# althonos/pyrodigal

Hardware: AMD Instinct MI355X
Metric: Mbp/sec gene-called (meta mode) (higher is better)
Workload: dtype f64; 1 GPU; 100000x20kbp_gc30-70_meta; contigs=100000, bases=2000000000, models=16, contigs_rank0=100000, sub_batch_contigs=6250, contexts_per_gpu=4, genes_all_ranks=2908995, steps_issued=a join of the contexts and a gather per step

## Files before the change

pyrodigal_amd/csrc/finder.hip:

```cpp
#include "pga_internal.h"
#include "pipeline.h"
#include "dpw_core.h"
#include "dev_common.h"
#include "find_plan.h"

#include <math.h>
#include <stdio.h>
#include <stdlib.h>
#include <string.h>

#include <algorithm>
#include <atomic>
#include <chrono>
#include <condition_variable>
#include <functional>
#include <limits>
#include <map>
#include <memory>
#include <mutex>
#include <new>
#include <thread>
#include <type_traits>
#include <unordered_map>

// ... 451 lines not shown
    int64_t out_off;
    int64_t dp_off;
    int64_t fin_off;
    int64_t topo_off;
    int32_t n;
    int32_t _pad;
};
struct GcPtrs { const float* p[4]; };
struct OutArrays {
    int32_t* ndx; int32_t* stop_val; uint8_t* type; int8_t* strand; float* gc_cont;
    uint8_t* edge_dp; double* cscore_dp; double* sscore_dp; double* rscore_dp; double* uscore_dp; double* tscore_dp;
    int32_t* star_ptr; int32_t* traceb; int8_t* ov_mark; double* score;
    uint8_t* edge; double* cscore; double* sscore; double* rscore; double* uscore; double* tscore; double* mot_score;
    int32_t* mot_ndx; uint8_t* rbs; uint8_t* mot_len; uint8_t* mot_spacer; uint8_t* mot_spacendx;
    int32_t direct;
    const int32_t* g_ndx[4]; const int32_t* g_stop_val[4]; const uint8_t* g_type[4]; const int8_t* g_strand[4];
    const uint8_t* c_edge; const double* c_cscore; const double* c_rscore; const double* c_uscore; const double* c_tscore;
    const int32_t* c_star_ptr; const double* d_score;
};

__global__ void __launch_bounds__(256)
k_gather_winners(const WinDesc* __restrict__ wd, int n_win, int64_t out_begin, int64_t total, GroupArrays ga, ChainArrays ca,
                 DpBuffers dp, OutArrays o, const int lean ) {
    __shared__ int s_w0;
    const int64_t blk0 = out_begin + (int64_t)blockIdx.x * blockDim.x;
    const int64_t g = blk0 + threadIdx.x;
    int lo = block_search_le([&](const int k) { return wd[k].out_off; }, n_win, blk0, &s_w0);
    if (g >= out_begin + total) return;
    while (lo + 1 < n_win && wd[lo + 1].out_off <= g) lo++;
    const WinDesc w = wd[lo];
    const int i = (int)(g - w.out_off);
    const int64_t t = w.topo_off + i, a = w.dp_off + i, f = w.fin_off + i;
    if (o.direct) { o.sscore_dp[g] = ca.sscore[a]; o.traceb[g] = dp.traceb[a]; o.ov_mark[g] = dp.ov_mark[a]; return; }
    o.ndx[g] = ga.ndx[t]; o.stop_val[g] = ga.stop_val[t]; o.type[g] = ga.type[t]; o.strand[g] = ga.strand[t];
    o.edge_dp[g] = ca.edge[a]; o.cscore_dp[g] = ca.cscore[a]; o.sscore_dp[g] = ca.sscore[a]; o.rscore_dp[g] = ca.rscore[a];
    o.uscore_dp[g] = ca.uscore[a]; o.tscore_dp[g] = ca.tscore[a];
    o.star_ptr[3 * g] = ca.star_ptr[3 * a]; o.star_ptr[3 * g + 1] = ca.star_ptr[3 * a + 1]; o.star_ptr[3 * g + 2] = ca.star_ptr[3 * a + 2];
    o.traceb[g] = dp.traceb[a]; o.ov_mark[g] = dp.ov_mark[a]; o.score[g] = dp.score[a];
    if (lean) return;
    o.gc_cont[g] = ga.gc_cont[t];
    o.edge[g] = ca.edge[f]; o.cscore[g] = ca.cscore[f]; o.sscore[g] = ca.sscore[f]; o.rscore[g] = ca.rscore[f];
    o.uscore[g] = ca.uscore[f]; o.tscore[g] = ca.tscore[f]; o.mot_score[g] = ca.mot_score[f]; o.mot_ndx[g] = ca.mot_ndx[f];
    o.rbs[2 * g] = ca.rbs[2 * f]; o.rbs[2 * g + 1] = ca.rbs[2 * f + 1];
    o.mot_len[g] = ca.mot_len[f]; o.mot_spacer[g] = ca.mot_spacer[f]; o.mot_spacendx[g] = ca.mot_spacendx[f];
}

struct GeneNodeAttr {
    double cscore, sscore, rscore, uscore, tscore, mot_score;
    float gc_cont; int32_t mot_ndx;
    uint8_t edge, rbs0, rbs1, mot_len, mot_spacer, _pad[3];
};
__global__ void __launch_bounds__(256)
k_gather_gene_nodes(const int64_t* __restrict__ idx, int n, OutArrays o, GeneNodeAttr* __restrict__ out) {
    const int t = blockIdx.x * blockDim.x + threadIdx.x;
    if (t >= n) return;
    const int64_t g = idx[t];
    GeneNodeAttr a;
    a.cscore = o.cscore[g]; a.sscore = o.sscore[g]; a.rscore = o.rscore[g]; a.uscore = o.uscore[g]; a.tscore = o.tscore[g];
    a.mot_score = o.mot_score[g]; a.gc_cont = o.gc_cont[g]; a.mot_ndx = o.mot_ndx[g];
    a.edge = o.edge[g]; a.rbs0 = o.rbs[2 * g]; a.rbs1 = o.rbs[2 * g + 1]; a.mot_len = o.mot_len[g]; a.mot_spacer = o.mot_spacer[g];
    a._pad[0] = a._pad[1] = a._pad[2] = 0;
    out[t] = a;
}

__device__ inline NodeView node_view(const TailDesc& d, const OutArrays& o, int32_t* tracef, uint8_t* elim) {
    const int64_t oo = d.out_off;
    if (o.direct) {
        const int64_t t = d.topo_off, a = d.dp_off; const int g = d.group;
        return NodeView{d.n, o.g_ndx[g] + t, o.g_stop_val[g] + t, o.g_type[g] + t, o.g_strand[g] + t, o.c_edge + a,
                        const_cast<double*>(o.c_cscore) + a, o.sscore_dp + oo, o.c_rscore + a, o.c_uscore + a, o.c_tscore + a,
                        o.c_star_ptr + 3 * a, o.traceb + oo, tracef + oo, o.ov_mark + oo, o.d_score + a, elim + oo};
    }
    return NodeView{d.n, o.ndx + oo, o.stop_val + oo, o.type + oo, o.strand + oo, o.edge_dp + oo,
                    o.cscore_dp + oo, o.sscore_dp + oo, o.rscore_dp + oo, o.uscore_dp + oo, o.tscore_dp + oo,
                    o.star_ptr + 3 * oo, o.traceb + oo, tracef + oo, o.ov_mark + oo, o.score + oo, elim + oo};
}

__global__ void __launch_bounds__(64)
k_tail_path(const TailDesc* __restrict__ td, int n_contigs, OutArrays o, int32_t* tracef, uint8_t* elim, int32_t* __restrict__ path,
            GeneRec* __restrict__ genes, int32_t* __restrict__ n_genes) {
    const int i = blockIdx.x * blockDim.x + threadIdx.x;
    if (i >= n_contigs) return;
    const TailDesc d = td[i];
    int ng = 0;
    if (d.n > 0 && d.mx >= 0) {
        NodeView v = node_view(d, o, tracef, elim);
        int32_t* pl = path + d.out_off;
        const int cnt = untangle(v, d.mx, pl);
        if (v.traceb[d.mx] != -1) {
            eliminate_bad_genes(v, pl, cnt, d.st_wt);
            ng = extract_genes(v, pl, cnt, genes + d.gene_off);
        }
    }
    n_genes[i] = ng;
}

__device__ inline int contig_of_slot(const TailDesc* __restrict__ td, int n_contigs, int64_t slot) {
    int lo = 0, hi = n_contigs - 1;
    while (lo < hi) { const int mid = (lo + hi + 1) >> 1; if (td[mid].gene_off <= slot) lo = mid; else hi = mid - 1; }
    return lo;
}

__global__ void __launch_bounds__(256)
k_tail_tweak(const TailDesc* __restrict__ td, int n_contigs, int64_t n_slots, OutArrays o, int32_t* tracef, uint8_t* elim,
             const GeneRec* __restrict__ orig, GeneRec* __restrict__ out, const int32_t* __restrict__ n_genes, int maxov,
             uint8_t* __restrict__ changed, int32_t* __restrict__ n_changed) {
    const int64_t slot = (int64_t)blockIdx.x * blockDim.x + threadIdx.x;
    if (slot >= n_slots) return;
    const int c = contig_of_slot(td, n_contigs, slot);
    const TailDesc d = td[c];
    const int g = (int)(slot - d.gene_off), ng = n_genes[c];
    if (g >= ng) return;
    const NodeView v = node_view(d, o, tracef, elim);
    const GeneRec* base = orig + d.gene_off;
    GeneRec cur = base[g];
    tweak_one(v, g > 0 ? &base[g - 1] : nullptr, cur, g < ng - 1 ? &base[g + 1] : nullptr, d.st_wt, maxov);
    out[slot] = cur;
    const bool moved = cur.start_ndx != base[g].start_ndx && v.strand[cur.start_ndx] == -1;
    changed[slot] = moved ? 1 : 0;
    if (moved) atomicAdd(&n_changed[c], 1);
}
__global__ void __launch_bounds__(256)
k_tail_init(int32_t* __restrict__ tracef, uint8_t* __restrict__ elim, const int64_t n_nodes, int32_t* __restrict__ nchanged, int32_t* __restrict__ ngenes ,
            const int n_contigs, int32_t* __restrict__ seg_cnt , const int n_segs) {
    const int64_t t = (int64_t)blockIdx.x * blockDim.x + threadIdx.x, stride = (int64_t)gridDim.x * blockDim.x;
    for (int64_t k = t; k <= n_nodes; k += stride) { tracef[k] = -1; elim[k] = 0; }
    for (int64_t k = t; k <= n_contigs; k += stride) { nchanged[k] = 0; if (ngenes != nullptr) ngenes[k] = 0; }
    if (seg_cnt != nullptr) for (int64_t k = t; k < n_segs; k += stride) seg_cnt[k] = 0;
}

__global__ void __launch_bounds__(1024)
k_gene_prefix(const int32_t* __restrict__ n_genes, int n_contigs, int32_t* __restrict__ gpre) {
    __shared__ int s_w[16];
    __shared__ int s_carry;
    const int t = threadIdx.x, lane = t & 63, w = t >> 6;
    if (t == 0) s_carry = 0;
    __syncthreads();
    for (int base = 0; base < n_contigs; base += 1024) {
        const int v = base + t < n_contigs ? n_genes[base + t] : 0;
        int inc = v;
#pragma unroll
        for (int o = 1; o < 64; o <<= 1) { const int x = __shfl_up(inc, o, 64); if (lane >= o) inc += x; }
        if (lane == 63) s_w[w] = inc;
        __syncthreads();
        int run = s_carry + inc - v;
        for (int k = 0; k < w; k++) run += s_w[k];
        if (base + t < n_contigs) gpre[base + t] = run;
        __syncthreads();
        if (t == 1023) s_carry = run + v;
        __syncthreads();
    }
    if (t == 0) gpre[n_contigs] = s_carry;
}
__global__ void __launch_bounds__(256)
k_tail_tweak_packed(const TailDesc* __restrict__ td, int n_contigs, OutArrays o, int32_t* tracef, uint8_t* elim,
                    const GeneRec* __restrict__ orig, GeneRec* __restrict__ out, const int32_t* __restrict__ n_genes, int maxov,
                    uint8_t* __restrict__ changed, int32_t* __restrict__ n_changed, const int32_t* __restrict__ gpre) {
    const int total = gpre[n_contigs];
    for (int q = blockIdx.x * blockDim.x + threadIdx.x; q < total; q += gridDim.x * blockDim.x) {
        int lo = 0, hi = n_contigs - 1;
        while (lo < hi) { const int mid = (lo + hi + 1) >> 1; if (gpre[mid] <= q) lo = mid; else hi = mid - 1; }
        const int c = lo, g = q - gpre[c], ng = n_genes[c];
        const TailDesc d = td[c];
        const NodeView v = node_view(d, o, tracef, elim);
        const GeneRec* base = orig + d.gene_off;
        GeneRec cur = base[g];
        tweak_one(v, g > 0 ? &base[g - 1] : nullptr, cur, g < ng - 1 ? &base[g + 1] : nullptr, d.st_wt, maxov);
        out[d.gene_off + g] = cur;
        const bool moved = cur.start_ndx != base[g].start_ndx && v.strand[cur.start_ndx] == -1;
        changed[d.gene_off + g] = moved ? 1 : 0;
        if (moved) atomicAdd(&n_changed[c], 1);
    }
}
__device__ void tweak_one_wave(const NodeView& v, const GeneRec* prev, GeneRec& cur, const GeneRec* next, double w, int maxov, const int lane) {
    const int nn = v.n;
    const int ndx = cur.start_ndx;
    const double sc = v.sscore[ndx] + v.cscore[ndx];
    double ig = 0.0;
    const bool prev_fwd = prev && v.strand[prev->start_ndx] == 1, prev_rev = prev && v.strand[prev->start_ndx] == -1;
    const bool next_fwd = next && v.strand[next->start_ndx] == 1, next_rev = next && v.strand[next->start_ndx] == -1;
    if (v.strand[ndx] == 1 && prev_fwd) ig = igm_same_h(v, prev->stop_ndx, ndx, w);
    if (v.strand[ndx] == 1 && prev_rev) ig = -0.15 * w;
    if (v.strand[ndx] == -1 && next_fwd) ig = -0.15 * w;
    if (v.strand[ndx] == -1 && next_rev) ig = igm_same_h(v, ndx, next->stop_ndx, w);
    int mi[2] = {-1, -1}; double ms[2] = {0, 0}, mg[2] = {0, 0};
    const int sv_ndx = v.stop_val[ndx];
    for (int base = ndx - 100; base < ndx + 100; base += 64) {
        const int j = base + lane;
        bool cand = j >= 0 && j < nn && j != ndx && j < ndx + 100;
        double tg = 0.0, cs = 0.0;
        if (cand) cand = !(is_stop_n(v, j) | (v.stop_val[j] != sv_ndx));
        if (cand) {
            const int sj = v.strand[j];
            if (sj == 1 && prev_fwd) {
                if (v.ndx[prev->stop_ndx] - v.ndx[j] > maxov) cand = false;
                else tg = igm_same_h(v, prev->stop_ndx, j, w);
            }
            if (cand && sj == 1 && prev_rev) { if (v.ndx[prev->start_ndx] - v.ndx[j] >= 0) cand = false; else tg = -0.15 * w; }
            if (cand && sj == -1 && next_fwd) { if (v.ndx[j] - v.ndx[next->start_ndx] >= 0) cand = false; else tg = -0.15 * w; }
            if (cand && sj == -1 && next_rev) {
                if (v.ndx[j] - v.ndx[next->stop_ndx] > maxov) cand = false;
                else tg = igm_same_h(v, j, next->stop_ndx, w);
            }
            if (cand) cs = v.cscore[j] + v.sscore[j];
        }
        unsigned long long m = __ballot(cand);
        while (m) {
            const int k = __builtin_ctzll(m);
            m &= m - 1ull;
            const int jk = base + k;
            const double csk = __shfl(cs, k, 64), tgk = __shfl(tg, k, 64);
            if (mi[0] == -1) { mi[0] = jk; ms[0] = csk; mg[0] = tgk; }
            else if (csk + tgk > ms[0]) { mi[1] = mi[0]; ms[1] = ms[0]; mg[1] = mg[0]; mi[0] = jk; ms[0] = csk; mg[0] = tgk; }
            else if (mi[1] == -1 || csk + tgk > ms[1]) { mi[1] = jk; ms[1] = csk; mg[1] = tgk; }
        }
    }
    for (int k = 0; k < 2; k++) {
        const int m = mi[k];
        if (m == -1) continue;
        if (v.tscore[m] < v.tscore[ndx] && ms[k] - v.tscore[m] >= sc - v.tscore[ndx] + w && v.rscore[m] > v.rscore[ndx] &&
            v.uscore[m] > v.uscore[ndx] && v.cscore[m] > v.cscore[ndx] && abs(v.ndx[m] - v.ndx[ndx]) > 15) {
            ms[k] += v.tscore[ndx] - v.tscore[m];
        } else if (abs(v.ndx[m] - v.ndx[ndx]) <= 15 && v.rscore[m] + v.tscore[m] > v.rscore[ndx] + v.tscore[ndx] &&
                   v.edge[ndx] == 0 && v.edge[m] == 0) {
            if (v.cscore[ndx] > v.cscore[m]) ms[k] += v.cscore[ndx] - v.cscore[m];
            if (v.uscore[ndx] > v.uscore[m]) ms[k] += v.uscore[ndx] - v.uscore[m];
            if (ig > mg[k]) ms[k] += ig - mg[k];
        } else ms[k] = -1000.0;
    }
    int pick = -1;
    for (int k = 0; k < 2; k++) {
        if (mi[k] == -1) continue;
        if (pick == -1 && ms[k] + mg[k] > sc + ig) pick = k;
        else if (pick >= 0 && ms[k] + mg[k] > ms[pick] + mg[pick]) pick = k;
    }
    if (pick != -1 && v.strand[mi[pick]] == 1) { cur.start_ndx = mi[pick]; cur.begin = v.ndx[mi[pick]] + 1; }
    else if (pick != -1 && v.strand[mi[pick]] == -1) { cur.start_ndx = mi[pick]; cur.end = v.ndx[mi[pick]] + 1; }
}

__global__ void __launch_bounds__(256)
k_tail_tweak_wave(const TailDesc* __restrict__ td, int n_contigs, OutArrays o, int32_t* tracef, uint8_t* elim,
                  const GeneRec* __restrict__ orig, GeneRec* __restrict__ out, const int32_t* __restrict__ n_genes, int maxov,
                  uint8_t* __restrict__ changed, int32_t* __restrict__ n_changed) {
    const int c = blockIdx.y, lane = threadIdx.x & 63;
    const int g = blockIdx.x * 4 + (threadIdx.x >> 6), ng = n_genes[c];
    if (g >= ng) return;
    const TailDesc d = td[c];
    const NodeView v = node_view(d, o, tracef, elim);
    const GeneRec* base = orig + d.gene_off;
    GeneRec cur = base[g];
    GeneRec prev{}, nxt{};
    if (g > 0) prev = base[g - 1];
    if (g < ng - 1) nxt = base[g + 1];
    tweak_one_wave(v, g > 0 ? &prev : nullptr, cur, g < ng - 1 ? &nxt : nullptr, d.st_wt, maxov, lane);
    if (lane != 0) return;
    out[d.gene_off + g] = cur;
    const bool moved = cur.start_ndx != base[g].start_ndx && v.strand[cur.start_ndx] == -1;
    changed[d.gene_off + g] = moved ? 1 : 0;
    if (moved) atomicAdd(&n_changed[c], 1);
}

#define PGA_FIX_MAXWIN 4096
__global__ void __launch_bounds__(1024)
k_tail_tweak_fixup(const TailDesc* __restrict__ td, int n_contigs, OutArrays o, int32_t* tracef, uint8_t* elim,
                   const GeneRec* __restrict__ orig, const GeneRec* __restrict__ par_all, const int32_t* __restrict__ n_genes, int maxov,
                   const uint8_t* __restrict__ ch0_all, const int32_t* __restrict__ n_changed, GeneRec* __restrict__ fin_all,
                   uint8_t* __restrict__ chf_all) {
    __shared__ uint8_t s_redone[PGA_FIX_MAXWIN];
    const int c = blockIdx.x, lane = threadIdx.x & 63, wave = threadIdx.x >> 6, nwaves = blockDim.x >> 6;
    if (c >= n_contigs) return;
    const TailDesc d = td[c];
    const int ng = n_genes[c];
    const GeneRec* ob = orig + d.gene_off; const GeneRec* par = par_all + d.gene_off; const uint8_t* ch0 = ch0_all + d.gene_off;
    GeneRec* fin = fin_all + d.gene_off; uint8_t* chf = chf_all + d.gene_off;
    for (int g = threadIdx.x; g < ng; g += blockDim.x) { fin[g] = par[g]; chf[g] = ch0[g]; }
    if (n_changed[c] == 0 || ng < 2) return;
    __threadfence_block();
    __syncthreads();
    const NodeView v = node_view(d, o, tracef, elim);
    const int nwin = (ng - 1 + 63) >> 6;
    auto run_window = [&](const int w, const bool assume) -> bool {
        const int g0 = 1 + (w << 6), g1 = min(ng, g0 + 64);
        const int g = g0 + lane;
        if (!assume) {
            if (g < g1) { fin[g] = par[g]; chf[g] = ch0[g]; }
            __builtin_amdgcn_fence(__ATOMIC_RELEASE, "workgroup");
            __builtin_amdgcn_fence(__ATOMIC_ACQUIRE, "workgroup");
        }
        const int pf = g < g1 ? ((lane == 0 && !assume) ? chf[g - 1] : ch0[g - 1]) : 0;
        unsigned long long mask = __ballot(pf != 0);
        bool last = false;
        while (mask) {
            const int k = __builtin_ctzll(mask);
            mask &= mask - 1ull;
            const int gg = g0 + k;
            GeneRec cur = ob[gg];
            const GeneRec prev = (k == 0 && assume) ? par[gg - 1] : fin[gg - 1];
            GeneRec nxt{};
            if (gg < ng - 1) nxt = ob[gg + 1];
            tweak_one_wave(v, &prev, cur, gg < ng - 1 ? &nxt : nullptr, d.st_wt, maxov, lane);
            const int nf = cur.start_ndx != ob[gg].start_ndx && v.strand[cur.start_ndx] == -1;
            if (lane == 0) { fin[gg] = cur; chf[gg] = (uint8_t)nf; }
            __builtin_amdgcn_fence(__ATOMIC_RELEASE, "workgroup");
            __builtin_amdgcn_fence(__ATOMIC_ACQUIRE, "workgroup");
            if (gg + 1 < g1) { if (nf) mask |= 1ull << (k + 1); else mask &= ~(1ull << (k + 1)); }
            if (gg == g1 - 1) last = true;
        }
        return last;
    };
    if (nwin <= PGA_FIX_MAXWIN) {
        for (int w = wave; w < nwin; w += nwaves) { const bool r = run_window(w, true); if (lane == 0) s_redone[w] = r; }
        __threadfence_block();
        __syncthreads();
        if (wave == 0)
            for (int w = 1; w < nwin; w++)
                if (s_redone[w - 1]) { const bool r = run_window(w, false); if (lane == 0) s_redone[w] = r; __builtin_amdgcn_wave_barrier(); }
    } else if (wave == 0) {
        for (int w = 0; w < nwin; w++) run_window(w, false);
    }
}

__global__ void __launch_bounds__(256)
k_emit_genes(const TailDesc* __restrict__ td, int n_contigs, int64_t n_slots, OutArrays o, const GeneRec* __restrict__ fin,
             const int32_t* __restrict__ n_genes, const int64_t* __restrict__ gene_begin, int single, pga_gene* __restrict__ out,
             const int lean, ChainArrays ca, GcPtrs gcs) {
    const int64_t slot = (int64_t)blockIdx.x * blockDim.x + threadIdx.x;
    if (slot >= n_slots) return;
    const int c = contig_of_slot(td, n_contigs, slot);
    const TailDesc d = td[c];
    const int g = (int)(slot - d.gene_off);
    if (g >= n_genes[c]) return;
    const GeneRec gr = fin[slot];
    const int64_t sn = d.out_off + gr.start_ndx, en = d.out_off + gr.stop_ndx;
    pga_gene G;
    memset(&G, 0, sizeof G);
    G.contig = c; G.begin = gr.begin; G.end = gr.end; G.start_ndx = gr.start_ndx; G.stop_ndx = gr.stop_ndx;
    if (o.direct) {
        const int64_t ts = d.topo_off + gr.start_ndx, as = d.dp_off + gr.start_ndx, ae = d.dp_off + gr.stop_ndx;
        const int64_t fs = d.fin_off + gr.start_ndx, fe = d.fin_off + gr.stop_ndx;
        G.strand = o.g_strand[d.group][ts];
        const uint8_t se = single ? o.c_edge[as] : ca.edge[fs], ee = single ? o.c_edge[ae] : ca.edge[fe];
        G.partial_begin = G.strand == 1 ? se : ee; G.partial_end = G.strand == 1 ? ee : se;
        G.start_type = se ? 3 : o.g_type[d.group][ts];
        G.rbs[0] = ca.rbs[2 * fs]; G.rbs[1] = ca.rbs[2 * fs + 1];
        G.mot_len = ca.mot_len[fs]; G.mot_spacer = ca.mot_spacer[fs]; G.mot_ndx = ca.mot_ndx[fs]; G.mot_score = ca.mot_score[fs];
        G.gc_cont = gcs.p[d.group][ts];
        G.cscore = single ? o.c_cscore[as] : ca.cscore[fs]; G.sscore = single ? o.sscore_dp[sn] : ca.sscore[fs];
        G.rscore = single ? o.c_rscore[as] : ca.rscore[fs]; G.uscore = single ? o.c_uscore[as] : ca.uscore[fs];
        G.tscore = single ? o.c_tscore[as] : ca.tscore[fs];
        out[gene_begin[c] + g] = G;
        return;
    }
    G.strand = o.strand[sn];
    if (lean) {
        const int64_t fs = d.fin_off + gr.start_ndx, fe = d.fin_off + gr.stop_ndx;
        const uint8_t se = single ? o.edge_dp[sn] : ca.edge[fs], ee = single ? o.edge_dp[en] : ca.edge[fe];
        G.partial_begin = G.strand == 1 ? se : ee; G.partial_end = G.strand == 1 ? ee : se;
        G.start_type = se ? 3 : o.type[sn];
        G.rbs[0] = ca.rbs[2 * fs]; G.rbs[1] = ca.rbs[2 * fs + 1];
        G.mot_len = ca.mot_len[fs]; G.mot_spacer = ca.mot_spacer[fs]; G.mot_ndx = ca.mot_ndx[fs]; G.mot_score = ca.mot_score[fs];
        G.gc_cont = gcs.p[d.group][d.topo_off + gr.start_ndx];
        G.cscore = single ? o.cscore_dp[sn] : ca.cscore[fs]; G.sscore = single ? o.sscore_dp[sn] : ca.sscore[fs];
        G.rscore = single ? o.rscore_dp[sn] : ca.rscore[fs]; G.uscore = single ? o.uscore_dp[sn] : ca.uscore[fs];
        G.tscore = single ? o.tscore_dp[sn] : ca.tscore[fs];
        out[gene_begin[c] + g] = G;
        return;
    }
    const uint8_t se = single ? o.edge_dp[sn] : o.edge[sn], ee = single ? o.edge_dp[en] : o.edge[en];
    G.partial_begin = G.strand == 1 ? se : ee; G.partial_end = G.strand == 1 ? ee : se;
    G.start_type = se ? 3 : o.type[sn];
    G.rbs[0] = o.rbs[2 * sn]; G.rbs[1] = o.rbs[2 * sn + 1];
    G.mot_len = o.mot_len[sn]; G.mot_spacer = o.mot_spacer[sn]; G.mot_ndx = o.mot_ndx[sn]; G.mot_score = o.mot_score[sn];
    G.gc_cont = o.gc_cont[sn];
    G.cscore = single ? o.cscore_dp[sn] : o.cscore[sn]; G.sscore = single ? o.sscore_dp[sn] : o.sscore[sn];
    G.rscore = single ? o.rscore_dp[sn] : o.rscore[sn]; G.uscore = single ? o.uscore_dp[sn] : o.uscore[sn];
    G.tscore = single ? o.tscore_dp[sn] : o.tscore[sn];
    out[gene_begin[c] + g] = G;
}

__global__ void __launch_bounds__(256)
k_cover_genes(const pga_gene* __restrict__ genes, int64_t n_genes, const ContigDesc* __restrict__ ct, int n_contigs, uint32_t* __restrict__ bits) {
    const int64_t g = (int64_t)blockIdx.x * 4 + (threadIdx.x >> 6);
    const int lane = threadIdx.x & 63;
    if (g >= n_genes) return;
    const int c = genes[g].contig;
    if (c < 0 || c >= n_contigs) return;
    const int32_t b = max(genes[g].begin, 1), e = min(genes[g].end, ct[c].len);
    if (b > e) return;
    const int64_t b0 = ct[c].base + b - 1, b1 = ct[c].base + e - 1;
    const int64_t w0 = b0 >> 5, w1 = b1 >> 5;
    for (int64_t w = w0 + lane; w <= w1; w += 64) {
        uint32_t m = 0xffffffffu;
        if (w == w0) m &= 0xffffffffu << (b0 & 31);
        if (w == w1) m &= 0xffffffffu >> (31 - (b1 & 31));
        atomicOr(&bits[w], m);
    }
}

__global__ void __launch_bounds__(256)
k_count_cover(const uint32_t* __restrict__ bits, const ContigDesc* __restrict__ ct, int64_t* __restrict__ coding) {
    __shared__ int64_t part[4];
    const int c = blockIdx.x;
    const int64_t lo = ct[c].base, len = ct[c].len;
    int64_t n = 0;
    if (len > 0) {
        const int64_t hi = lo + len - 1, w0 = lo >> 5, w1 = hi >> 5;
        for (int64_t w = w0 + threadIdx.x; w <= w1; w += blockDim.x) {
            uint32_t m = bits[w];
            if (w == w0) m &= 0xffffffffu << (lo & 31);
            if (w == w1) m &= 0xffffffffu >> (31 - (hi & 31));
            n += __popc(m);
        }
    }
    for (int d = 32; d > 0; d >>= 1) n += __shfl_down(n, d, 64);
    if ((threadIdx.x & 63) == 0) part[threadIdx.x >> 6] = n;
    __syncthreads();
    if (threadIdx.x == 0) coding[c] = part[0] + part[1] + part[2] + part[3];
}

#include "tail.inl"

struct ResultOwner {
    pga_result pub;
    std::vector<pga_contig_result> contigs;
    std::vector<pga_gene> genes;
    pga_gene* pin_genes = nullptr; size_t pin_cap = 0, pin_n = 0;
    std::vector<pga_nodes> nodes;
    std::vector<int32_t> mask_off, masks;
    bool has_masks = false;
    std::vector<void*> blocks;
    ~ResultOwner() {
        for (void* b : blocks) free(b);
        if (pin_genes != nullptr) cache_put_result(pin_genes, pin_cap);
    }
    pga_gene* gene_records(const size_t n, const bool pageable ) {
        const size_t bytes = n * sizeof(pga_gene);
        if (bytes < ((size_t)256 << 10) || pageable) { genes.resize(n); return genes.data(); }
        size_t cap = 0;
        void* p = cache_take(1, -1, bytes, &cap, 8);
        if (p == nullptr) {
            cap = (bytes + ((size_t)1 << 20)) & ~(((size_t)1 << 20) - 1);
            if (hipHostMalloc(&p, cap, hipHostMallocDefault) != hipSuccess) { (void)hipGetLastError(); genes.resize(n); return genes.data(); }
        }
        pin_genes = (pga_gene*)p; pin_cap = cap; pin_n = n;
        return pin_genes;
    }
};

int alloc_nodes(ResultOwner* R, pga_nodes& N, const int n) {
    memset(&N, 0, sizeof N);
    N.n = n;
    const size_t bytes = (size_t)n * (4 * 8 + 10 + 4 + 8 * 7) + 8 * 32;
    char* blk = (char*)calloc(1, bytes);
// ... 1292 lines not shown
        if (NC < 4) nt = 1;
        if (nt == 1) fn(); else f->pool.run(fn, nt);
    };
    run_parallel(worker);
    if (P.want_nodes && out_nodes > 0)
        HT(c, hipMemcpyAsync(o.sscore_dp, h.sscore_dp, sizeof(double) * (size_t)out_nodes, hipMemcpyHostToDevice, st));
    tm->mark("host_tail");
    std::vector<int32_t> n_genes((size_t)NC);
    for (int i = 0; i < NC; i++) n_genes[i] = (int32_t)cg[i].size();
    const int64_t ngenes = contig_results(n_genes.data(), nullptr);
    R->genes.resize((size_t)ngenes);
    PINBUF(h_gidx, int64_t, "h_gidx", 2 * ngenes + 1);
    PINBUF(h_attr, GeneNodeAttr, "h_attr", 2 * ngenes + 1);
    if (ngenes > 0) {
        DEVBUF(d_gidx, int64_t, "d_gidx", 2 * ngenes + 1);
        DEVBUF(d_attr, GeneNodeAttr, "d_attr", 2 * ngenes + 1);
        for (int i = 0; i < NC; i++) {
            int64_t gi = R->contigs[i].gene_begin;
            for (const GeneRec& gr : cg[i]) { h_gidx[2 * gi] = out_off[i] + gr.start_ndx; h_gidx[2 * gi + 1] = out_off[i] + gr.stop_ndx; gi++; }
        }
        HT(c, hipMemcpyAsync(d_gidx, h_gidx, sizeof(int64_t) * 2 * ngenes, hipMemcpyHostToDevice, st));
        hipLaunchKernelGGL(k_gather_gene_nodes, dim3((unsigned)((2 * ngenes + 255) / 256)), dim3(256), 0, st, d_gidx, (int)(2 * ngenes), o, d_attr);
        HT(c, hipMemcpyAsync(h_attr, d_attr, sizeof(GeneNodeAttr) * 2 * ngenes, hipMemcpyDeviceToHost, st));
        if (const int rc = sync()) return rc;
    }
    tm->mark("gene_attrs");
    std::atomic<int> next2(0);
    auto filler = [&]() {
        for (;;) {
            const int i = next2.fetch_add(1);
            if (i >= NC) break;
            const int k = win_chain[i];
            if (k < 0) continue;
            const int64_t oo = out_off[i];
            const bool single = !P.meta;
            int64_t gi = R->contigs[i].gene_begin;
            for (const GeneRec& gr : cg[i]) {
                pga_gene& G = R->genes[(size_t)gi];
                const GeneNodeAttr& as = h_attr[2 * gi]; const GeneNodeAttr& ae = h_attr[2 * gi + 1];
                gi++;
                memset(&G, 0, sizeof G);
                const int64_t sn = oo + gr.start_ndx, en = oo + gr.stop_ndx;
                G.contig = i; G.begin = gr.begin; G.end = gr.end; G.start_ndx = gr.start_ndx; G.stop_ndx = gr.stop_ndx;
                G.strand = h.strand[sn];
                const uint8_t se = single ? h.edge_dp[sn] : as.edge, ee = single ? h.edge_dp[en] : ae.edge;
                G.partial_begin = G.strand == 1 ? se : ee; G.partial_end = G.strand == 1 ? ee : se;
                G.start_type = se ? 3 : h.type[sn];
                G.rbs[0] = as.rbs0; G.rbs[1] = as.rbs1;
                G.mot_len = as.mot_len; G.mot_spacer = as.mot_spacer; G.mot_ndx = as.mot_ndx; G.mot_score = as.mot_score;
                G.gc_cont = as.gc_cont;
                G.cscore = single ? h.cscore_dp[sn] : as.cscore; G.sscore = single ? h.sscore_dp[sn] : as.sscore;
                G.rscore = single ? h.rscore_dp[sn] : as.rscore; G.uscore = single ? h.uscore_dp[sn] : as.uscore;
                G.tscore = single ? h.tscore_dp[sn] : as.tscore;
            }
        }
    };
    run_parallel(filler);
    if (coding) {
        std::vector<std::pair<int32_t, int32_t>> iv;
        for (int i = 0; i < NC; i++) {
            iv.clear();
            const int32_t len = batch->ct[i].len;
            for (const GeneRec& gr : cg[i]) {
                const int32_t b = std::max<int32_t>(gr.begin, 1), e = std::min<int32_t>(gr.end, len);
                if (b <= e) iv.emplace_back(b, e);
            }
            std::sort(iv.begin(), iv.end());
            int64_t n = 0; int32_t hi = 0;
            for (const auto& x : iv) {
                if (x.second <= hi) continue;
                n += x.second - std::max(x.first - 1, hi);
                hi = x.second;
            }
            coding[i] = n;
        }
    }
    return PGA_OK;
}

struct TailBufs {
    TailDesc* d_td; int32_t* d_tracef; uint8_t* d_elim; GeneRec* d_gene0; GeneRec* d_gene1; GeneRec* d_gene2; int32_t* d_ngenes;
    int32_t* d_path; uint8_t* d_changed; int32_t* d_nchanged;
    int64_t n_slots; unsigned init_blocks;
};

int FindCall::launch_tail_paths(const TailBufs& t) {
    bool tail_inited = false;
    for (int i = 0; i < NC; i++) if (win_chain[i] >= 0 && chains[win_chain[i]].n > 0) segs.push_back(TpSeg{out_off[i], chains[win_chain[i]].n, i});
    std::sort(segs.begin(), segs.end(), [](const TpSeg& a, const TpSeg& b) { return a.off < b.off; });
    if (!segs.empty() && out_nodes > 0) {
        if (out_nodes >= (1ll << 30)) { c->err = "pga_find_genes: more than 2^30 nodes in the winning chains of one batch"; return PGA_EINVAL; }
        int levels = 1;
        while ((1ll << levels) < max_n) levels++;
        const unsigned nblk = (unsigned)((out_nodes + 255) / 256);
        const bool tp_steps = kn.tp_steps;
        const bool tp_one = max_n <= TP_SMALL_MAX && !tp_steps;
        const int64_t tpn = tp_one ? 0 : out_nodes;
        DEVBUF(tp_seg, TpSeg, "tp_seg", segs.size()) DEVBUF(tp_up, int32_t, "tp_up", (size_t)2 * tpn)
        DEVBUF(tp_mark, uint8_t, "tp_mark", tpn) DEVBUF(tp_slots, int32_t, "tp_slots", tpn)
        DEVBUF(tp_ins, int32_t, "tp_ins", 2 * tpn) DEVBUF(tp_excl, int32_t, "tp_excl", tpn + 1)
        DEVBUF(tp_bsum, int32_t, "tp_bsum", nblk + 1) DEVBUF(tp_cnt, int32_t, "tp_cnt", segs.size())
        HT(c, hipMemcpyAsync(tp_seg, segs.data(), sizeof(TpSeg) * segs.size(), hipMemcpyHostToDevice, st));
        hipLaunchKernelGGL(k_tail_init, dim3(t.init_blocks), dim3(256), 0, st, t.d_tracef, t.d_elim, out_nodes, t.d_nchanged, t.d_ngenes, NC,
                           tp_one ? (int32_t*)nullptr : tp_cnt, (int)segs.size());
        tail_inited = true;
        const TpWork tw{tp_seg, (int)segs.size(), out_nodes, levels, tp_up, tp_mark, tp_slots, tp_ins, tp_excl, tp_bsum, tp_cnt};
        const dim3 grid(nblk), blk(256);
        if (tp_one) {
            const int cap = (int)((max_n + 63) & ~63ll);
            hipLaunchKernelGGL(k_tp_small, dim3((unsigned)segs.size()), dim3(max_n <= 2048 ? 64 : 256), sizeof(int32_t) * 3 * (size_t)cap, st, tw, t.d_td, o,
                               t.d_tracef, t.d_elim, t.d_gene0, t.d_ngenes, cap);
        } else {
            hipLaunchKernelGGL(k_tp_init, grid, blk, 0, st, tw, t.d_td, o);
            {
                const bool j8 = kn.tp_jump8;
                int k = 0;
                for (int left = levels; left > 0; k++) {
                    const int32_t* in = tp_up + (size_t)(k & 1) * out_nodes; int32_t* outp = tp_up + (size_t)((k + 1) & 1) * out_nodes;
                    if (j8 && left >= 3) { hipLaunchKernelGGL(k_tp_jump8, grid, blk, 0, st, tw, in, outp); left -= 3; }
                    else { hipLaunchKernelGGL(k_tp_jump, grid, blk, 0, st, tw, in, outp); left -= 1; }
                }
            }
            hipLaunchKernelGGL(k_tp_slots, grid, blk, 0, st, tw, t.d_td, o);
            hipLaunchKernelGGL(k_tp_scan1, grid, blk, 0, st, tw);
            hipLaunchKernelGGL(k_tp_scan2, dim3(1), dim3(1024), 0, st, tw, (int)nblk);
            hipLaunchKernelGGL(k_tp_scan3, grid, blk, 0, st, tw);
            hipLaunchKernelGGL(k_tp_fill, grid, blk, 0, st, tw, o, t.d_path);
            hipLaunchKernelGGL(k_tp_link, grid, blk, 0, st, tw, o, t.d_path, t.d_tracef);
            hipLaunchKernelGGL(k_tp_elim_a, grid, blk, 0, st, tw, t.d_td, o, t.d_path);
            hipLaunchKernelGGL(k_tp_elim_b, grid, blk, 0, st, tw, t.d_td, o, t.d_path, t.d_elim);
            if (max_n >= 32768 && segs.size() <= 64 && !kn.tp_extract_one) {
                const int chunks = (max_n + 1023) / 1024;
                DEVBUF(tp_xsum, TpChunkSum, "tp_xsum", (size_t)chunks * segs.size() + 1);
                const dim3 xg((unsigned)chunks, (unsigned)segs.size());
                hipLaunchKernelGGL(k_tp_extract_sum, xg, dim3(1024), 0, st, tw, t.d_td, o, t.d_path, t.d_elim, tp_xsum, chunks);
                hipLaunchKernelGGL(k_tp_extract_chunk, xg, dim3(1024), 0, st, tw, t.d_td, o, t.d_path, t.d_elim, (const TpChunkSum*)tp_xsum, chunks, t.d_gene0,
                                   t.d_ngenes);
            } else
                hipLaunchKernelGGL(k_tp_extract, dim3((unsigned)segs.size()), dim3(max_n >= 32768 ? 1024 : 256), 0, st, tw, t.d_td, o, t.d_path, t.d_elim,
                                   t.d_gene0, t.d_ngenes);
        }
    }
    if (!tail_inited) hipLaunchKernelGGL(k_tail_init, dim3(t.init_blocks), dim3(256), 0, st, t.d_tracef, t.d_elim, out_nodes, t.d_nchanged, t.d_ngenes, NC, (int32_t*)nullptr, 0);
    return PGA_OK;
}

int FindCall::launch_tail_tweaks(TailBufs& t) {
    if (max_n >= 32768 && NC <= 1024)
        hipLaunchKernelGGL(k_tail_tweak_wave, dim3((unsigned)((max_n / 2 + 2 + 3) / 4), (unsigned)NC), dim3(256), 0, st, t.d_td, NC, o, t.d_tracef,
                           t.d_elim, t.d_gene0, t.d_gene1, t.d_ngenes, P.max_overlap, t.d_changed, t.d_nchanged);
    else if (NC >= 256 && !kn.tweak_slots) {
        DEVBUF(d_gpre, int32_t, "d_gene_prefix", NC + 2);
        hipLaunchKernelGGL(k_gene_prefix, dim3(1), dim3(1024), 0, st, t.d_ngenes, NC, d_gpre);
        hipLaunchKernelGGL(k_tail_tweak_packed, dim3(1024), dim3(256), 0, st, t.d_td, NC, o, t.d_tracef, t.d_elim, t.d_gene0, t.d_gene1, t.d_ngenes,
                           P.max_overlap, t.d_changed, t.d_nchanged, d_gpre);
    } else
        hipLaunchKernelGGL(k_tail_tweak, dim3((unsigned)((t.n_slots + 255) / 256)), dim3(256), 0, st, t.d_td, NC, t.n_slots, o, t.d_tracef, t.d_elim,
                           t.d_gene0, t.d_gene1, t.d_ngenes, P.max_overlap, t.d_changed, t.d_nchanged);
    DEVSET(t.d_gene2, GeneRec, "d_gene2", t.n_slots + 1);
    DEVBUF(d_chfin, uint8_t, "d_chfin", t.n_slots + 1);
    hipLaunchKernelGGL(k_tail_tweak_fixup, dim3(NC), dim3(max_n >= 32768 ? 1024 : 128), 0, st, t.d_td, NC, o, t.d_tracef, t.d_elim, t.d_gene0, t.d_gene1,
                       t.d_ngenes, P.max_overlap, t.d_changed, t.d_nchanged, t.d_gene2, d_chfin);
    return PGA_OK;
}

int FindCall::run_device_tail(const bool par_tail) {
    tm->mark("gather");
    tdv.resize(NC);
    int64_t n_slots = 0;
    for (int i = 0; i < NC; i++) {
        const int k = win_chain[i];
        TailDesc& d = tdv[i];
        d.out_off = k >= 0 ? out_off[i] : 0; d.gene_off = n_slots;
        d.n = k >= 0 ? chains[k].n : 0; d.mx = k >= 0 ? h_maxidx[k] : -1;
        d.st_wt = k >= 0 ? c->models[chains[k].model].st_wt : 0.0;
        d.fin_off = k >= 0 ? fin_off[i] : 0; d.topo_off = k >= 0 ? chains[k].topo_off : 0;
        d.group = k >= 0 ? chains[k].group : 0; d._pad = 0;
        d.dp_off = k >= 0 ? chains[k].off : 0;
        n_slots += d.n / 2 + 2;
    }
    DEVBUF(d_td, TailDesc, "d_taildesc", NC + 1);
    DEVBUF(d_tracef, int32_t, "d_tracef", out_nodes + 1);
    DEVBUF(d_elim, uint8_t, "d_elim", out_nodes + 1);
    DEVBUF(d_gene0, GeneRec, "d_gene0", n_slots + 1);
    DEVBUF(d_gene1, GeneRec, "d_gene1", n_slots + 1);
    DEVBUF(d_ngenes, int32_t, "d_ngenes", NC + 1);
    DEVBUF(d_gbegin, int64_t, "d_gbegin", NC + 1);
    PINBUF(h_ngenes, int32_t, "h_ngenes", NC + 1);
    PINBUF(h_gbegin, int64_t, "h_gbegin", NC + 1);
    HT(c, hipMemcpyAsync(d_td, tdv.data(), sizeof(TailDesc) * NC, hipMemcpyHostToDevice, st));
    DEVBUF(d_path, int32_t, "d_path", out_nodes + 1);
    DEVBUF(d_changed, uint8_t, "d_changed", n_slots + 1);
    DEVBUF(d_nchanged, int32_t, "d_nchanged", NC + 1);
    TailBufs t{d_td, d_tracef, d_elim, d_gene0, d_gene1, nullptr, d_ngenes, d_path, d_changed, d_nchanged, n_slots,
               (unsigned)std::min<int64_t>(2048, (std::max<int64_t>(out_nodes, NC) + 256) / 256)};
    if (!par_tail) {
        hipLaunchKernelGGL(k_tail_init, dim3(t.init_blocks), dim3(256), 0, st, d_tracef, d_elim, out_nodes, d_nchanged, (int32_t*)nullptr, NC, (int32_t*)nullptr, 0);
        hipLaunchKernelGGL(k_tail_path, dim3((NC + 63) / 64), dim3(64), 0, st, d_td, NC, o, d_tracef, d_elim, d_path, d_gene0, d_ngenes);
    } else if (const int rc = launch_tail_paths(t)) return rc;
    if (const int rc = launch_tail_tweaks(t)) return rc;
    HT(c, hipMemcpyAsync(h_ngenes, d_ngenes, sizeof(int32_t) * NC, hipMemcpyDeviceToHost, st));
    if (const int rc = sync()) return rc;
    tm->mark("tail");
    const int64_t ngenes = contig_results(h_ngenes, h_gbegin);
    pga_gene* const genes_out = coding || keep ? nullptr : R->gene_records((size_t)ngenes, kn.pageable_results);
    pga_gene* d_genes = nullptr;
    if (ngenes > 0) {
        DEVBUF(d_genes_out, pga_gene, keep ? keep->buf : "d_genes_out", ngenes + 1);
        d_genes = d_genes_out;
        HT(c, hipMemcpyAsync(d_gbegin, h_gbegin, sizeof(int64_t) * NC, hipMemcpyHostToDevice, st));
        GcPtrs gcs{};
        for (int g = 0; g < NG; g++) gcs.p[g] = ga[g].gc_cont;
        hipLaunchKernelGGL(k_emit_genes, dim3((unsigned)((n_slots + 255) / 256)), dim3(256), 0, st, d_td, NC, n_slots, o, t.d_gene2, d_ngenes,
                           d_gbegin, P.meta ? 0 : 1, d_genes, lean_gather ? 1 : 0, ca, gcs);
        if (genes_out) HT(c, hipMemcpyAsync(genes_out, d_genes, sizeof(pga_gene) * (size_t)ngenes, hipMemcpyDeviceToHost, st));
        if (keep) { keep->d_genes = d_genes; keep->n_genes = ngenes; }
    }
    if (coding) {
        const int64_t words = total / 32 + 2;
        DEVBUF(d_cover, uint32_t, "d_cover", words);
        DEVBUF(d_coding, int64_t, "d_coding", NC + 1);
        PINBUF(h_coding, int64_t, "h_coding", NC + 1);
        HT(c, hipMemsetAsync(d_cover, 0, sizeof(uint32_t) * (size_t)words, st));
        if (ngenes > 0)
            hipLaunchKernelGGL(k_cover_genes, dim3((unsigned)((ngenes + 3) / 4)), dim3(256), 0, st, d_genes, ngenes, d_ct, NC, d_cover);
        hipLaunchKernelGGL(k_count_cover, dim3((unsigned)NC), dim3(256), 0, st, d_cover, d_ct, d_coding);
        HT(c, hipMemcpyAsync(h_coding, d_coding, sizeof(int64_t) * NC, hipMemcpyDeviceToHost, st));
        if (const int rc = sync()) return rc;
        memcpy(coding, h_coding, sizeof(int64_t) * NC);
    }
    if (P.want_nodes == 1 && out_nodes > 0) {
        tracef.resize((size_t)out_nodes + 1); elim.resize((size_t)out_nodes + 1);
        HT(c, hipMemcpyAsync(h.ndx, o.ndx, arena_all, hipMemcpyDeviceToHost, st));
        HT(c, hipMemcpyAsync(tracef.data(), d_tracef, sizeof(int32_t) * (size_t)out_nodes, hipMemcpyDeviceToHost, st));
        HT(c, hipMemcpyAsync(elim.data(), d_elim, (size_t)out_nodes, hipMemcpyDeviceToHost, st));
    }
    if (const int rc = stop_clock()) return rc;
    tm->mark("genes+d2h");
    return PGA_OK;
}

int FindCall::copy_out_nodes() {
    R->nodes.resize(NC);
    for (int i = 0; i < NC; i++) {
        pga_nodes& N = R->nodes[i];
        memset(&N, 0, sizeof N);
        const int k = win_chain[i];
        if (k < 0) continue;
        const int n = chains[k].n; const int64_t oo = out_off[i];
        const bool single = !P.meta;
        if (int rc = alloc_nodes(R, N, n)) return rc;
        copy_node_topology(N, n, h.ndx + oo, h.stop_val + oo, h.type + oo, h.strand + oo, (single ? h.edge_dp : h.edge) + oo);
        const double* const src64[6] = {(single ? h.cscore_dp : h.cscore) + oo, (single ? h.sscore_dp : h.sscore) + oo, (single ? h.rscore_dp : h.rscore) + oo,
                                        (single ? h.uscore_dp : h.uscore) + oo, (single ? h.tscore_dp : h.tscore) + oo, h.mot_score + oo};
        copy_node_scores(N, n, src64, h.mot_ndx + oo, h.rbs + 2 * oo, h.mot_len + oo, h.mot_spacer + oo, h.mot_spacendx + oo, h.gc_cont + oo);
        if (single) {
            memcpy(N.score, h.score + oo, 8 * (size_t)n); memcpy(N.traceb, h.traceb + oo, 4 * (size_t)n); memcpy(N.tracef, tracef.data() + oo, 4 * (size_t)n);
            memcpy(N.ov_mark, h.ov_mark + oo, n); memcpy(N.elim, elim.data() + oo, n); memcpy(N.star_ptr, h.star_ptr + 3 * oo, 12 * (size_t)n);
        } else reset_dp_fields(N, n);
    }
    return PGA_OK;
}

void FindCall::keep_device_nodes() {
    DevNodes& D = c->dev_nodes;
    D.off.assign(NC, 0); D.n.assign(NC, 0); D.len.resize(NC);
    for (int i = 0; i < NC; i++) {
        D.len[i] = batch->ct[i].len;
        if (win_chain[i] >= 0) { D.off[i] = out_off[i]; D.n[i] = chains[win_chain[i]].n; }
    }
    D.total = out_nodes;
    const bool single = !P.meta;
    D.a = DevNodeArrays{o.ndx, o.stop_val, o.type, o.strand, o.gc_cont,
                        single ? o.edge_dp : o.edge, single ? o.cscore_dp : o.cscore, single ? o.sscore_dp : o.sscore,
                        single ? o.rscore_dp : o.rscore, single ? o.uscore_dp : o.uscore, single ? o.tscore_dp : o.tscore,
                        o.mot_score, o.mot_ndx, o.rbs, o.mot_len, o.mot_spacer};
    D.batch = batch;
    D.contigs = R->contigs.data();
}

}

static int find_impl(const Knobs& kn, pga_ctx* c, const pga_batch* batch, const pga_params* pp, const int stage, const int tt_override, pga_result** out,
                     const int32_t* model_of_contig, const int32_t* tt_of_contig, int64_t* coding = nullptr, GeneKeep* keep = nullptr) {
    FindCall s;
    s.stage = stage; s.tt_override = tt_override; s.model_of_contig = model_of_contig; s.tt_of_contig = tt_of_contig; s.coding = coding; s.keep = keep;
    if (const int rc = s.check_call(kn, c, batch, pp, out)) return rc;
    StageTimer tm(kn.timing);
    s.tm = &tm;
    if (s.NC > 0 && s.total > 0) {
        if (const int rc = s.run_sequence_and_masks()) return rc;
        if (stage == PGA_STAGE_SEQUENCE) return s.return_sequence_stage(out);
        if (const int rc = s.run_extract()) return rc;
        tm.mark("extract+sync");
        if (const int rc = s.place_nodes()) return rc;
        if (const int rc = s.plan_chains()) return rc;
        if (const int rc = s.plan_connection_scoring()) return rc;
        if (const int rc = s.upload_plan()) return rc;
        tm.mark("plan+alloc");
        if (const int rc = s.score_groups()) return rc;
        if (stage != 0) return s.return_stage_nodes(out);
        if (const int rc = s.score_connections()) return rc;
        tm.mark("score+dp+sync");
        s.pick_winners();
        if (const int rc = s.rescore_winners()) return rc;
        tm.mark("winners+rescore_launch");
        if (const int rc = s.gather_winners()) return rc;
        const bool device_tail = kn.tail != Knobs::host;
// ... 194 lines not shown
```

Measured before the change: 20770 Mbp/s.

## Parallelize packed start tweak across lane groups with compacted candidate scan

Changes the packed tail-tweak kernel from one thread per gene to a group of 8 lanes per gene, using a templated group-width version of the wavefront tweak routine. The candidate scan first pre-filters the ±100 node window by stop/frame validity, then compacts the surviving candidates so each round only evaluates real candidates. The contig lookup becomes a group-cooperative k-ary search instead of a per-thread binary search. This is meant to cut divergence and serial work per gene in the tweak step, in exchange for more ballot/shuffle overhead and a larger grid. The existing 64-lane callers also pick up the compacted scan.

```diff
diff --git a/pyrodigal_amd/csrc/finder.hip b/pyrodigal_amd/csrc/finder.hip
--- a/pyrodigal_amd/csrc/finder.hip
+++ b/pyrodigal_amd/csrc/finder.hip
@@ -627,27 +627,11 @@
     }
     if (t == 0) gpre[n_contigs] = s_carry;
 }
-__global__ void __launch_bounds__(256)
-k_tail_tweak_packed(const TailDesc* __restrict__ td, int n_contigs, OutArrays o, int32_t* tracef, uint8_t* elim,
-                    const GeneRec* __restrict__ orig, GeneRec* __restrict__ out, const int32_t* __restrict__ n_genes, int maxov,
-                    uint8_t* __restrict__ changed, int32_t* __restrict__ n_changed, const int32_t* __restrict__ gpre) {
-    const int total = gpre[n_contigs];
-    for (int q = blockIdx.x * blockDim.x + threadIdx.x; q < total; q += gridDim.x * blockDim.x) {
-        int lo = 0, hi = n_contigs - 1;
-        while (lo < hi) { const int mid = (lo + hi + 1) >> 1; if (gpre[mid] <= q) lo = mid; else hi = mid - 1; }
-        const int c = lo, g = q - gpre[c], ng = n_genes[c];
-        const TailDesc d = td[c];
-        const NodeView v = node_view(d, o, tracef, elim);
-        const GeneRec* base = orig + d.gene_off;
-        GeneRec cur = base[g];
-        tweak_one(v, g > 0 ? &base[g - 1] : nullptr, cur, g < ng - 1 ? &base[g + 1] : nullptr, d.st_wt, maxov);
-        out[d.gene_off + g] = cur;
-        const bool moved = cur.start_ndx != base[g].start_ndx && v.strand[cur.start_ndx] == -1;
-        changed[d.gene_off + g] = moved ? 1 : 0;
-        if (moved) atomicAdd(&n_changed[c], 1);
-    }
-}
+template <int W>
 __device__ void tweak_one_wave(const NodeView& v, const GeneRec* prev, GeneRec& cur, const GeneRec* next, double w, int maxov, const int lane) {
+    static_assert(W == 8 || W == 16 || W == 32 || W == 64, "a group is a power-of-two share of the wavefront");
+    constexpr unsigned long long GROUP = W == 64 ? ~0ull : (1ull << (W & 63)) - 1ull;
+    const int gl = lane & (W - 1), g0 = lane - gl;
     const int nn = v.n;
     const int ndx = cur.start_ndx;
     const double sc = v.sscore[ndx] + v.cscore[ndx];
@@ -660,11 +644,32 @@
     if (v.strand[ndx] == -1 && next_rev) ig = igm_same_h(v, ndx, next->stop_ndx, w);
     int mi[2] = {-1, -1}; double ms[2] = {0, 0}, mg[2] = {0, 0};
     const int sv_ndx = v.stop_val[ndx];
-    for (int base = ndx - 100; base < ndx + 100; base += 64) {
-        const int j = base + lane;
-        bool cand = j >= 0 && j < nn && j != ndx && j < ndx + 100;
+    constexpr int ROUNDS = (200 + W - 1) / W;
+    unsigned pass = 0;
+#pragma unroll
+    for (int r = 0; r < ROUNDS; r++) {
+        const int j = ndx - 100 + W * r + gl;
+        const int jj = j < 0 ? 0 : (j >= nn ? nn - 1 : j);
+        const bool ok = !(is_stop_n(v, jj) | (v.stop_val[jj] != sv_ndx)) && j >= 0 && j < nn && j != ndx && j < ndx + 100;
+        pass |= (unsigned)ok << r;
+    }
+    int t0 = 0, total;
+    do {
+        const int t = t0 + gl;
+        int j = -1, cnt = 0;
+#pragma unroll
+        for (int r = 0; r < ROUNDS; r++) {
+            unsigned long long m = (__ballot((pass >> r) & 1u) >> g0) & GROUP;
+            const int pc = __popcll(m);
+            if (t >= cnt && t < cnt + pc) {
+                for (int s = t - cnt; s > 0; s--) m &= m - 1ull;
+                j = ndx - 100 + W * r + __builtin_ctzll(m);
+            }
+            cnt += pc;
+        }
+        total = cnt;
+        bool cand = j >= 0;
         double tg = 0.0, cs = 0.0;
-        if (cand) cand = !(is_stop_n(v, j) | (v.stop_val[j] != sv_ndx));
         if (cand) {
             const int sj = v.strand[j];
             if (sj == 1 && prev_fwd) {
@@ -679,17 +684,18 @@
             }
             if (cand) cs = v.cscore[j] + v.sscore[j];
         }
-        unsigned long long m = __ballot(cand);
+        unsigned long long m = (__ballot(cand) >> g0) & GROUP;
         while (m) {
             const int k = __builtin_ctzll(m);
             m &= m - 1ull;
-            const int jk = base + k;
-            const double csk = __shfl(cs, k, 64), tgk = __shfl(tg, k, 64);
+            const int jk = __shfl(j, k, W);
+            const double csk = __shfl(cs, k, W), tgk = __shfl(tg, k, W);
             if (mi[0] == -1) { mi[0] = jk; ms[0] = csk; mg[0] = tgk; }
             else if (csk + tgk > ms[0]) { mi[1] = mi[0]; ms[1] = ms[0]; mg[1] = mg[0]; mi[0] = jk; ms[0] = csk; mg[0] = tgk; }
             else if (mi[1] == -1 || csk + tgk > ms[1]) { mi[1] = jk; ms[1] = csk; mg[1] = tgk; }
         }
-    }
+        t0 += W;
+    } while (t0 < total);
     for (int k = 0; k < 2; k++) {
         const int m = mi[k];
         if (m == -1) continue;
@@ -727,12 +733,54 @@
     GeneRec prev{}, nxt{};
     if (g > 0) prev = base[g - 1];
     if (g < ng - 1) nxt = base[g + 1];
-    tweak_one_wave(v, g > 0 ? &prev : nullptr, cur, g < ng - 1 ? &nxt : nullptr, d.st_wt, maxov, lane);
+    tweak_one_wave<64>(v, g > 0 ? &prev : nullptr, cur, g < ng - 1 ? &nxt : nullptr, d.st_wt, maxov, lane);
     if (lane != 0) return;
     out[d.gene_off + g] = cur;
     const bool moved = cur.start_ndx != base[g].start_ndx && v.strand[cur.start_ndx] == -1;
     changed[d.gene_off + g] = moved ? 1 : 0;
     if (moved) atomicAdd(&n_changed[c], 1);
+}
+
+#ifndef PGA_TWEAK_LANES
+#define PGA_TWEAK_LANES 8
+#endif
+template <int W>
+__device__ inline int group_search_le(const int32_t* __restrict__ pre, int n, const int q, const int lane) {
+    constexpr unsigned long long GROUP = W == 64 ? ~0ull : (1ull << (W & 63)) - 1ull;
+    const int gl = lane & (W - 1), g0 = lane - gl;
+    int lo = 0;
+    while (n > 1) {
+        const int step = (n + W - 1) / W;
+        const bool ok = gl * step < n && pre[lo + gl * step] <= q;
+        const int cnt = __popcll((__ballot(ok) >> g0) & GROUP);
+        lo += (cnt - 1) * step;
+        n = min(step, n - (cnt - 1) * step);
+    }
+    return lo;
+}
+template <int W>
+__global__ void __launch_bounds__(256)
+k_tail_tweak_packed(const TailDesc* __restrict__ td, int n_contigs, OutArrays o, int32_t* tracef, uint8_t* elim,
+                    const GeneRec* __restrict__ orig, GeneRec* __restrict__ out, const int32_t* __restrict__ n_genes, int maxov,
+                    uint8_t* __restrict__ changed, int32_t* __restrict__ n_changed, const int32_t* __restrict__ gpre) {
+    constexpr int PER_WG = 256 / W;
+    const int total = gpre[n_contigs], lane = threadIdx.x & 63;
+    for (int q = blockIdx.x * PER_WG + threadIdx.x / W; q < total; q += gridDim.x * PER_WG) {
+        const int c = group_search_le<W>(gpre, n_contigs, q, lane), g = q - gpre[c], ng = n_genes[c];
+        const TailDesc d = td[c];
+        const NodeView v = node_view(d, o, tracef, elim);
+        const GeneRec* base = orig + d.gene_off;
+        GeneRec cur = base[g];
+        GeneRec prev{}, nxt{};
+        if (g > 0) prev = base[g - 1];
+        if (g < ng - 1) nxt = base[g + 1];
+        tweak_one_wave<W>(v, g > 0 ? &prev : nullptr, cur, g < ng - 1 ? &nxt : nullptr, d.st_wt, maxov, lane);
+        if ((lane & (W - 1)) != 0) continue;
+        out[d.gene_off + g] = cur;
+        const bool moved = cur.start_ndx != base[g].start_ndx && v.strand[cur.start_ndx] == -1;
+        changed[d.gene_off + g] = moved ? 1 : 0;
+        if (moved) atomicAdd(&n_changed[c], 1);
+    }
 }
 
 #define PGA_FIX_MAXWIN 4096
@@ -773,7 +821,7 @@
             const GeneRec prev = (k == 0 && assume) ? par[gg - 1] : fin[gg - 1];
             GeneRec nxt{};
             if (gg < ng - 1) nxt = ob[gg + 1];
-            tweak_one_wave(v, &prev, cur, gg < ng - 1 ? &nxt : nullptr, d.st_wt, maxov, lane);
+            tweak_one_wave<64>(v, &prev, cur, gg < ng - 1 ? &nxt : nullptr, d.st_wt, maxov, lane);
             const int nf = cur.start_ndx != ob[gg].start_ndx && v.strand[cur.start_ndx] == -1;
             if (lane == 0) { fin[gg] = cur; chf[gg] = (uint8_t)nf; }
             __builtin_amdgcn_fence(__ATOMIC_RELEASE, "workgroup");
@@ -2372,8 +2420,9 @@
     else if (NC >= 256 && !kn.tweak_slots) {
         DEVBUF(d_gpre, int32_t, "d_gene_prefix", NC + 2);
         hipLaunchKernelGGL(k_gene_prefix, dim3(1), dim3(1024), 0, st, t.d_ngenes, NC, d_gpre);
-        hipLaunchKernelGGL(k_tail_tweak_packed, dim3(1024), dim3(256), 0, st, t.d_td, NC, o, t.d_tracef, t.d_elim, t.d_gene0, t.d_gene1, t.d_ngenes,
-                           P.max_overlap, t.d_changed, t.d_nchanged, d_gpre);
+        const unsigned wgs = (unsigned)std::min<int64_t>(4096, (t.n_slots + 256 / PGA_TWEAK_LANES - 1) / (256 / PGA_TWEAK_LANES));
+        hipLaunchKernelGGL(k_tail_tweak_packed<PGA_TWEAK_LANES>, dim3(std::max(1u, wgs)), dim3(256), 0, st, t.d_td, NC, o, t.d_tracef, t.d_elim, t.d_gene0,
+                           t.d_gene1, t.d_ngenes, P.max_overlap, t.d_changed, t.d_nchanged, d_gpre);
     } else
         hipLaunchKernelGGL(k_tail_tweak, dim3((unsigned)((t.n_slots + 255) / 256)), dim3(256), 0, st, t.d_td, NC, t.n_slots, o, t.d_tracef, t.d_elim,
                            t.d_gene0, t.d_gene1, t.d_ngenes, P.max_overlap, t.d_changed, t.d_nchanged);
```

Result: slower. 20150 Mbp/s (-3.0%).
